# NeurAI-Lab/biHomE

Hardware: AMD Instinct MI355X
Metric: training image-pairs/s (128x128 patch, bs=64 per GPU, full step: fwd+bwd+Adam) (higher is better)
Workload: dtype f32

## Files before the change

### bihome_amd/csrc/conv3x3.hip

```cpp
#include "common.h"
#include "conv3x3_args.h"
#include <type_traits>

#ifndef C3_X3_PIPE
#define C3_X3_PIPE 0
#endif

#ifndef C3_BN32_WAVES
#define C3_BN32_WAVES 2
#endif

#ifdef BH_TUNING
__device__ unsigned long long g_c3_ts[8 * 16384];
#define C3_STAMP(tile, k) do { if (a.dbg_ts && threadIdx.x == 0 && (tile) < 16384) { g_c3_ts[(tile) * 8 + (k)] = wall_clock64();          \
        if ((k) == 1 || (k) == 2) g_c3_ts[(tile) * 8 + 4 + (k)] = __builtin_readcyclecounter(); } } while (0)
#else
#define C3_STAMP(tile, k) do { } while (0)
#endif

constexpr int C3_HALO_BYTES = 8 * 200 * 16;
constexpr int C3_B_BYTES = 8192;
constexpr int C3_LDS_BYTES = 2 * C3_HALO_BYTES + 2 * C3_B_BYTES;

template <int BN, int SUBT, int TM, bool MAP4 = false>
// ... 635 lines not shown
            for (int r = 0; r < 16; ++r) acc[i][r] = __builtin_ldexpf(acc[i][r], f16_kout);
    }
    double s1, s2;
    int img, g;
    c3_epilogue<BN, SUBT, TM, MAP4>(a, acc, bx, n0, wm, wn, wh, l31, kh2, s1, s2, img, g, AMX);
    if (a.bn_sums) {
        if (a.stat_acc) { S1 += s1; S2 += s2; Sbx = bx; if (g < Sg) { Sg = g; Simg = img; } }
        else c3_stats_merge<BN, 0>(a, smem, s1, s2, img, g, bx, n0, wave, lane, tid);
    }
#ifdef BH_TUNING
    if (a.dbg_ts) asm volatile("s_waitcnt vmcnt(0)" ::: "memory");
#endif
    __syncthreads();
    C3_STAMP(bx * gridDim.y + blockIdx.y, 3);
    }
    if (a.bn_sums && a.stat_acc) c3_stats_merge<BN, 0>(a, smem, S1, S2, Simg, Sg, Sbx, n0, wave, lane, tid);
    if (a.amax_out) {
        const float m = wave_max(AMX);
        if (lane == 0) atomicMax(a.amax_out + ((blockIdx.x * 4 + wave) % BH_AMAX_SLOTS) * BH_AMAX_STRIDE, __builtin_bit_cast(unsigned, m));
    }
}

constexpr int C3_MIN_BLOCKS = 256;
BH_KNOB(g_c3_noload, 0); BH_KNOB(g_c3_dbg_nch, -1); BH_KNOB(g_c3_subt, 2); BH_KNOB(g_c3_tpb, 2); BH_KNOB(g_c3_stamp, 0); BH_KNOB(g_c3_desync, 0); BH_KNOB(g_c3_walk32, 1); BH_KNOB(g_c3_pc, 1); BH_KNOB(g_c3_wt64, 512); BH_KNOB(g_c3_wt32, 512);
#ifdef BH_TUNING
extern "C" int bh_debug_read_c3_stamps(unsigned long long* out, int n) {
    if (n > 16384) n = 16384;
    return (int)hipMemcpyFromSymbol(out, HIP_SYMBOL(g_c3_ts), (size_t)n * 8 * sizeof(unsigned long long), 0, hipMemcpyDeviceToHost);
}
void bh_conv3x3_tune(int disable, int min_blocks) {
    (void)min_blocks;
    if (disable >= 500 && disable < 1000) { g_c3_stamp = disable - 500; return; }
    if (disable >= 200 && disable < 264) { g_c3_desync = disable - 200; return; }
    if (disable == 300 || disable == 301) { g_c3_walk32 = disable - 300; return; }
    if (disable >= 2000 && disable < 6000) { g_c3_wt64 = disable - 2000; return; }
    if (disable >= 6000 && disable < 10000) { g_c3_wt32 = disable - 6000; return; }
    if (disable == 310 || disable == 311) { g_c3_pc = disable - 310; return; }
    if (disable <= -100) { g_c3_dbg_nch = -100 - disable - 1; return; }
    if (disable >= 400 && disable < 464) { g_c3_noload = disable - 400; return; }
    if (disable >= 20 && disable < 24) { g_c3_tpb = disable - 20; return; }
    if (disable >= 11 && disable <= 13) { g_c3_subt = disable - 10; return; }
}
#endif

int bh_conv3x3_try(const float* src, const float* w, const float* bias, float* out, const bh_conv_desc* d, int dgrad,
                   int accumulate, hipStream_t stream, int* taken, double* bn_sums, int groups, const float* res, int relu,
                   const bh_bn_reduce* bnr, const bh_bn_in* bni) {
    *taken = 0;
    if ((d->route & BH_ROUTE_GENERIC_CONV) || d->transposed || d->kh != 3 || d->kw != 3 || d->stride != 1 || d->pad != 1 || d->in_nchw ||
        d->out_nchw || d->precision < 0 || d->precision > 4)
        return d->w_layout ? BH_E_UNSUPPORTED : 0;
    if (d->w_layout != 0 && ((d->w_layout == 2) != (d->precision == 2) || (d->w_layout == 3) != (d->precision == 3) ||
                             (d->w_layout == 4) != (d->precision == 4))) return BH_E_BADARG;
    if (d->w_layout == 4 && !d->a_bound) return BH_E_BADARG;
    const bool map4 = d->Hi == 4 && d->Wi == 4 && d->Ho == 4 && d->Wo == 4 && d->N % 4 == 0 && (d->w_layout >= 2 && d->w_layout <= 4) &&
                      d->Co % 64 == 0 && d->Ci % 64 == 0 && !bni && (!bn_sums || (groups >= 1 && d->N % groups == 0 && (d->N / groups) % 4 == 0));
    if (!map4 && (d->Hi % 8 || d->Wi % 8 || d->Ho != d->Hi || d->Wo != d->Wi)) return d->w_layout ? BH_E_UNSUPPORTED : 0;
    const int Kc = dgrad ? d->Co : d->Ci, Nn = dgrad ? d->Ci : d->Co;
    if (Kc % 32 || Nn % 32) return d->w_layout ? BH_E_UNSUPPORTED : 0;
    const int bn_tile = (Nn % 64) ? 32 : 64;
// ... 40 lines not shown
    if (bn_sums && !map4 && !(d->route & BH_ROUTE_C3_ONE_POSITION) && groups >= 1 && a.subtiles % (subt * groups) == 0) {
        const int ppg = a.subtiles / (subt * groups);
        int t = a.tpb;
        const long long wtarget = (x3 && bn_tile == 64) ? g_c3_wt64 : (x3 ? g_c3_wt32 : 2048);
        while (ppg % (t * 2) == 0 && (ppg / t > 1024 || (long long)(ppg / t) * groups * grid.y > wtarget) && t < 64) t *= 2;
        if (ppg % t == 0 && (t > 1 || a.tpb == 1)) {
            if (t != a.tpb) { a.tpb = t; grid.x = (a.gx_total + t - 1) / t; }
            a.stat_acc = 1;
        }
    }
    if (x3 && !map4 && a.tpb == 1 && !bn_sums && g_c3_walk32 && !(d->route & BH_ROUTE_C3_ONE_POSITION)) {
        const long long target = bn_tile == 32 ? 1024 : 512;
        int t = 1;
        while (a.gx_total % (t * 2) == 0 && (long long)(a.gx_total / (t * 2)) * grid.y >= target && t < 64) t *= 2;
        if (t > 1) { a.tpb = t; grid.x = a.gx_total / t; }
    }
    if (!(d->route & BH_ROUTE_HALO_SMALL) && (int)((map4 ? a.subtiles : (a.subtiles + 1) / 2) * grid.y) < (map4 ? C3_MIN_BLOCKS / 2 : C3_MIN_BLOCKS))
        return d->w_layout ? BH_E_UNSUPPORTED : 0;
    a.NW = Nn / 32;
    if (bni) {
        if (!x3 || dgrad || !bni->table || bni->groups < 1 || d->N % bni->groups || (long long)bni->groups * Kc * 8 > 4096) return BH_E_UNSUPPORTED;
        a.bni = bni->table; a.bni_relu = bni->relu; a.bni_groups = bni->groups; a.bni_ipg = d->N / bni->groups;
    }
    if (f16 && !map4 && bn_tile == 64 && !(d->route & (BH_ROUTE_C3_TILE_WG | BH_ROUTE_C3_ONE_SUBTILE | BH_ROUTE_C3_ONE_POSITION)) && g_c3_pc) {
        C3Args b = a;
        b.det = (d->route & BH_ROUTE_DETERMINISTIC) ? 1 : 0; b.dbg_noload = g_c3_noload; b.dbg_ts = g_c3_stamp;
        const int st = bh_conv3x3_pc_launch(b, dgrad, bni ? bni->table : nullptr, bni ? bni->groups : 0, bni ? bni->relu : 0, (d->route & BH_ROUTE_C3_PC) != 0, stream);
        if (st != BH_E_UNSUPPORTED) { if (st == BH_OK) *taken = 1; return st; }
    }
    if (bh_query("conv3x3_halo_kernel<%s,%d,%s,%d,%s,%s,%s,%d,%s,%s>", dgrad ? "true" : "false", bn_tile, bf16 ? "true" : "false", subt,
                 packed ? "true" : "false", x3 ? "true" : "false", bni ? "true" : "false", np, map4 ? "true" : "false", f16 ? "true" : "false")) {
        *taken = 1;
        return BH_OK;
    }
    static unsigned long long attr_devs = 0;
    typedef void (*kern_t)(C3Args);
#define C3_ROW(P) conv3x3_halo_kernel<false, 64, false, 2, P>, conv3x3_halo_kernel<true, 64, false, 2, P>,   \
                  conv3x3_halo_kernel<false, 32, false, 2, P>, conv3x3_halo_kernel<true, 32, false, 2, P>,   \
                  conv3x3_halo_kernel<false, 64, true, 2, P>,  conv3x3_halo_kernel<true, 64, true, 2, P>,    \
                  conv3x3_halo_kernel<false, 32, true, 2, P>,  conv3x3_halo_kernel<true, 32, true, 2, P>,    \
                  conv3x3_halo_kernel<false, 64, false, 1, P>, conv3x3_halo_kernel<true, 64, false, 1, P>,   \
                  conv3x3_halo_kernel<false, 64, true, 1, P>,  conv3x3_halo_kernel<true, 64, true, 1, P>
#define C3_XROW(NP_, F_) conv3x3_halo_kernel<false, 64, false, 2, true, true, false, NP_, false, F_>, conv3x3_halo_kernel<true, 64, false, 2, true, true, false, NP_, false, F_>,  \
                     conv3x3_halo_kernel<false, 32, false, 2, true, true, false, NP_, false, F_>, conv3x3_halo_kernel<true, 32, false, 2, true, true, false, NP_, false, F_>,  \
                     conv3x3_halo_kernel<false, 64, false, 1, true, true, false, NP_, false, F_>, conv3x3_halo_kernel<true, 64, false, 1, true, true, false, NP_, false, F_>,  \
                     conv3x3_halo_kernel<false, 64, false, 2, true, true, true, NP_, false, F_>, conv3x3_halo_kernel<false, 32, false, 2, true, true, true, NP_, false, F_>,   \
                     conv3x3_halo_kernel<false, 64, false, 1, true, true, true, NP_, false, F_>
// ... 148 lines not shown
```

### bihome_amd/csrc/conv3x3_pc.hip

```cpp
#include "conv3x3_args.h"
#include <type_traits>

namespace {
constexpr int PC_HPL = 200;
constexpr int PC_PS = PC_HPL * 16 + 32;
constexpr int PC_PIECE = 4 * PC_PS;
constexpr int PC_STAGE = 2 * PC_PIECE;
constexpr int PC_BTAP = 8192;
constexpr int PC_BROW = 3 * PC_BTAP;
constexpr int PC_OFF_B = 2 * PC_STAGE;
constexpr int PC_OFF_EPI = PC_OFF_B + 3 * PC_BROW;
constexpr int PC_EPI_BYTES = 128 * 64 * 4;
constexpr int PC_OFF_RED = PC_OFF_EPI + PC_EPI_BYTES;
constexpr int PC_RED_BYTES = 4 * 128 * 8;
constexpr int PC_LDS = PC_OFF_RED + PC_RED_BYTES;
constexpr unsigned PC_XOOB = 0x80000000u;

#ifdef BH_TUNING
__device__ unsigned long long g_pc_ts[12 * 160 * 2];
#define PC_BARRIER()                                                                                                    \
    do {                                                                                                                \
        const bool st_ = a.dbg_ts && blockIdx.x == (unsigned)(a.dbg_ts - 1) && (tid & 63) == 0;                        \
        if (st_ && pc_nb < 160) g_pc_ts[(wave * 160 + pc_nb) * 2] = __builtin_readcyclecounter();                       \
        asm volatile("s_waitcnt lgkmcnt(0)\n\ts_barrier" ::: "memory");                                                \
        if (st_ && pc_nb < 160) g_pc_ts[(wave * 160 + pc_nb) * 2 + 1] = __builtin_readcyclecounter();                   \
        ++pc_nb;                                                                                                        \
    } while (0)
#else
#define PC_BARRIER() asm volatile("s_waitcnt lgkmcnt(0)\n\ts_barrier" ::: "memory")
#endif
#ifndef PC_EMU
#define PC_EMU 0
#endif
#define PC_H_ASM 0
#define PC_BARRIER_VM() asm volatile("s_waitcnt vmcnt(0)\n\ts_waitcnt lgkmcnt(0)\n\ts_barrier" ::: "memory")

__device__ __forceinline__ unsigned pc_amax_reduce(unsigned v) {
#pragma unroll
    for (int off = 8; off > 0; off >>= 1) { const unsigned o = (unsigned)__shfl_xor((int)v, off, 64); v = o > v ? o : v; }
    return (unsigned)__builtin_amdgcn_readfirstlane((int)v);
}

__device__ __forceinline__ void pc_decode(const C3Args& a, int g, int& img, int& ty, int& tx) {
    if (a.tpi_shift >= 0) { img = g >> a.tpi_shift; const int t = g & (a.tiles_per_img - 1); ty = t >> a.tx_shift; tx = t & (a.tiles_x - 1); }
    else { img = g / a.tiles_per_img; const int t = g - img * a.tiles_per_img; ty = t / a.tiles_x; tx = t - ty * a.tiles_x; }
}

template <bool DGRAD, bool BNI, int EM>
__global__ void __launch_bounds__(768) conv3x3_pc_kernel(C3Args a) {
    extern __shared__ __attribute__((aligned(16))) char smem[];
    const int tid = threadIdx.x, lane = tid & 63;
    const int wave = __builtin_amdgcn_readfirstlane(tid >> 6);
    const int NY = a.Nn >> 6;
    const int total = a.gx_total * NY;
    const int wt0 = blockIdx.x * a.tpb;
    const int Tw = min(a.tpb, total - wt0);
    const int nch = a.Kc >> 5;
    const int K = Tw * nch;
    const int R = K * 3;
#ifdef BH_TUNING
    int pc_nb = 0;
#endif

    auto wait_vm = [&](int n) {
#define PC_W(k) case k: asm volatile("s_waitcnt vmcnt(" #k ")" ::: "memory"); break;
        switch (n < 0 ? 0 : (n > 48 ? 48 : n)) {
            PC_W(0) PC_W(1) PC_W(2) PC_W(3) PC_W(4) PC_W(5) PC_W(6) PC_W(7) PC_W(8) PC_W(9) PC_W(10) PC_W(11) PC_W(12) PC_W(13) PC_W(14) PC_W(15)
            PC_W(16) PC_W(17) PC_W(18) PC_W(19) PC_W(20) PC_W(21) PC_W(22) PC_W(23) PC_W(24) PC_W(25) PC_W(26) PC_W(27) PC_W(28) PC_W(29) PC_W(30)
            PC_W(31) PC_W(32) PC_W(33) PC_W(34) PC_W(35) PC_W(36) PC_W(37) PC_W(38) PC_W(39) PC_W(40) PC_W(41) PC_W(42) PC_W(43) PC_W(44) PC_W(45)
            PC_W(46) PC_W(47) PC_W(48)
        }
#undef PC_W
    };

    if (wave < 4) {
        const int l31 = lane & 31, kh2 = lane >> 5;
        const int wm = wave & 1, wn = wave >> 1;
        const int sr_ = c3_strip_row(l31 >> 2);
        const char* const aL = smem + kh2 * PC_PS + (wm * 100 + sr_ * 10 + (l31 & 3)) * 16;
        const char* const bL = smem + PC_OFF_B + wn * 4096 + lane * 16;
        int eoff[4];
#pragma unroll
        for (int rq = 0; rq < 4; ++rq) eoff[rq] = PC_OFF_EPI + ((wm * 64 + c3_strip_row(2 * rq + kh2) * 8) * 64 + wn * 32 + l31) * 4;
        uint4 FA0[2][2], FB0[2], FA1[2][2], FB1[2];
        f32x16 acc[2];
#ifdef BH_TUNING
        const int dbg = a.dbg_noload;
#else
        constexpr int dbg = 0;
#endif
#define PC_LD_A(A_, ap, s2, i_, pc_) A_[i_][pc_] = *reinterpret_cast<const uint4*>((ap) + (pc_) * PC_PIECE + 2 * (s2) * PC_PS + (i_) * 64)
#define PC_LD_B(B_, bp, s2, pc_) B_[pc_] = *reinterpret_cast<const uint4*>((bp) + ((pc_) * 2 + (s2)) * 1024)
#define PC_LOADH(A_, B_, ap, bp, s2)                                                                                    \
    do {                                                                                                                \
        PC_LD_A(A_, ap, s2, 0, 1); PC_LD_B(B_, bp, s2, 0); PC_LD_A(A_, ap, s2, 1, 1);                                   \
        PC_LD_A(A_, ap, s2, 0, 0); PC_LD_B(B_, bp, s2, 1); PC_LD_A(A_, ap, s2, 1, 0);                                   \
    } while (0)
#define PC_STEP(ACC, AV, BV, LD)                                                                                        \
    do {                                                                                                                \
        ACC = c3_mfma16<true>(AV, BV, ACC);                                                                             \
        LD;                                                                                                             \
        __builtin_amdgcn_sched_barrier(0);                                                                              \
    } while (0)
#define PC_HALF(UA, UB, LA, LB, ap, bp, s2)                                                                             \
    do {                                                                                                                \
        PC_STEP(acc[0], UA[0][1], UB[0], PC_LD_A(LA, ap, s2, 0, 1));                                                    \
        PC_STEP(acc[1], UA[1][1], UB[0], PC_LD_B(LB, bp, s2, 0));                                                       \
        PC_STEP(acc[0], UA[0][0], UB[1], PC_LD_A(LA, ap, s2, 1, 1));                                                    \
        PC_STEP(acc[1], UA[1][0], UB[1], PC_LD_A(LA, ap, s2, 0, 0));                                                    \
        PC_STEP(acc[0], UA[0][0], UB[0], PC_LD_B(LB, bp, s2, 1));                                                       \
        PC_STEP(acc[1], UA[1][0], UB[0], PC_LD_A(LA, ap, s2, 1, 0));                                                    \
    } while (0)
#define PC_HALF_PRE(UA, UB, LA, LB, ap, bp, s2)                                                                         \
    do {                                                                                                                \
        PC_LOADH(LA, LB, ap, bp, s2);                                                                                   \
        __builtin_amdgcn_sched_barrier(0);                                                                              \
        PC_STEP(acc[0], UA[0][1], UB[0], (void)0);                                                                      \
        PC_STEP(acc[1], UA[1][1], UB[0], (void)0);                                                                      \
        PC_STEP(acc[0], UA[0][0], UB[1], (void)0);                                                                      \
        PC_STEP(acc[1], UA[1][0], UB[1], (void)0);                                                                      \
        PC_STEP(acc[0], UA[0][0], UB[0], (void)0);                                                                      \
        PC_STEP(acc[1], UA[1][0], UB[0], (void)0);                                                                      \
    } while (0)
        PC_BARRIER();
        PC_LOADH(FA0, FB0, aL, bL, 0);
#if PC_EMU
        PC_LOADH(FA1, FB1, aL, bL, 1);
#undef PC_LD_B
#define PC_LD_B(B_, bp, s2, pc_) (void)0
#if PC_EMU >= 2
#undef PC_LD_A
#if PC_EMU == 2
#define PC_LD_A(A_, ap, s2, i_, pc_) (void)0
#else
#define PC_LD_A(A_, ap, s2, i_, pc_) do { if ((i_) == 0) A_[i_][pc_] = *reinterpret_cast<const uint4*>((ap) + (pc_) * PC_PIECE + 2 * (s2) * PC_PS + (i_) * 64); } while (0)
#endif
#endif
#endif
        int kap = 0;
        for (int ti = 0; ti < Tw; ++ti) {
#pragma unroll
            for (int i = 0; i < 2; ++i)
#pragma unroll
                for (int r = 0; r < 16; ++r) acc[i][r] = 0.0f;
            for (int c = 0; c < nch; ++c, ++kap) {
                const int par = kap & 1;
                const bool more = kap + 1 < K;
#pragma unroll
                for (int row = 0; row < 3; ++row) {
                    const char* const rp = aL + par * PC_STAGE + row * 160;
                    const char* const sp = bL + row * PC_BROW;
                    const char* const nrp = row < 2 ? rp + 160 : (more ? aL + (par ^ 1) * PC_STAGE : rp);
                    const char* const nsp = row < 2 ? sp + PC_BROW : bL;
                    if (dbg & 1) { PC_BARRIER(); continue; }
#pragma unroll
                    for (int t = 0; t < 3; ++t) {
                        if (t < 2) PC_HALF(FA0, FB0, FA1, FB1, rp + t * 16, sp + t * PC_BTAP, 1);
                        else {
                            PC_HALF_PRE(FA0, FB0, FA1, FB1, rp + t * 16, sp + t * PC_BTAP, 1);
                            PC_BARRIER();
                        }
                        if (t < 2) PC_HALF(FA1, FB1, FA0, FB0, rp + (t + 1) * 16, sp + (t + 1) * PC_BTAP, 0);
                        else PC_HALF(FA1, FB1, FA0, FB0, nrp, nsp, 0);
                    }
                }
            }
            asm volatile("s_nop 15\n\ts_nop 15" : "+v"(acc[0]), "+v"(acc[1]));
#pragma unroll
            for (int i = 0; i < 2; ++i)
#pragma unroll
                for (int r = 0; r < 16; ++r)
                    *reinterpret_cast<float*>(smem + eoff[r >> 2] + (4 * i + (r & 3)) * 256) = acc[i][r];
        }
        PC_BARRIER();
        PC_BARRIER();
        PC_BARRIER();
        PC_BARRIER();
#undef PC_HALF_PRE
#undef PC_HALF
#undef PC_STEP
#undef PC_LOADH
#undef PC_LD_A
#undef PC_LD_B
        return;
    }

    if (wave < 7) {
        __builtin_amdgcn_s_setprio(2);
        const int ht = tid - 256;
        const int plane = ht & 3;
        const __amdgpu_buffer_rsrc_t rsA = __builtin_amdgcn_make_buffer_rsrc(const_cast<float*>(a.Src), 0, a.src_bytes, 0x00020000);
        const __amdgpu_buffer_rsrc_t rsT = __builtin_amdgcn_make_buffer_rsrc(const_cast<float*>(BNI ? a.bni : a.Src), 0,
                                                                              BNI ? (unsigned)(a.bni_groups * a.Kc * 8) : 0u, 0x00020000);
        constexpr int NR = 5;
        const int lo0 = plane * PC_PS + (ht >> 2) * 16;
// ... 136 lines not shown
        PC_BARRIER();
        PC_BARRIER();
        PC_BARRIER();
#undef PC_H_ISSUE_ALL
#undef PC_H_CHUNK
        return;
    }

    if (wave < 8) {
        const __amdgpu_buffer_rsrc_t rsB = __builtin_amdgcn_make_buffer_rsrc(const_cast<float*>(a.Wt), 0, a.w_bytes, 0x00020000);
#ifdef BH_TUNING
        const bool doff = a.dbg_noload & 8;
#else
        constexpr bool doff = false;
#endif
        auto dma_num = [&](int r) {
            const int kp = r / 3, row = r - kp * 3, ti_ = kp / nch, c_ = kp - ti_ * nch;
            const int ny = (wt0 + ti_) / a.gx_total;
#pragma unroll
            for (int t = 0; t < 3; ++t)
#pragma unroll
                for (int piece = 0; piece < 8; ++piece) {
                    const unsigned so = (unsigned)(((c_ * 9 + row * 3 + t) * a.NW + ny * 2) * 4096 + piece * 1024);
                    __builtin_amdgcn_raw_ptr_buffer_load_lds(rsB, (lds_void_ptr)(smem + PC_OFF_B + row * PC_BROW + t * PC_BTAP + piece * 1024), 16,
                                                             (unsigned)lane * 16u, so, 0, 0);
                }
        };
        int pro = 0;
        if (!doff) { dma_num(0); if (R > 1) { dma_num(1); ++pro; } if (R > 2) { dma_num(2); ++pro; } }
        wait_vm(24 * pro);
        PC_BARRIER();
        for (int rho = 0; rho < R; ++rho) {
            int nd = 0;
            if (rho >= 1 && rho + 2 < R && !doff) { dma_num(rho + 2); nd = 24; }
            wait_vm(rho == 0 ? ((R > 2 && !doff) ? 24 : 0) : nd);
            PC_BARRIER();
        }
        PC_BARRIER();
        PC_BARRIER();
        PC_BARRIER();
        PC_BARRIER();
        return;
    }

    {
        __builtin_amdgcn_s_setprio(1);
        const int ew = wave - 8;
        const int cq = lane & 15, pl = lane >> 4;
        const __amdgpu_buffer_rsrc_t rsO = __builtin_amdgcn_make_buffer_rsrc(a.Out, 0, a.out_bytes, 0x00020000);
        const __amdgpu_buffer_rsrc_t rsR = __builtin_amdgcn_make_buffer_rsrc(const_cast<float*>(a.res ? a.res : a.Out), 0, a.out_bytes, 0x00020000);
        const __amdgpu_buffer_rsrc_t rsZ = __builtin_amdgcn_make_buffer_rsrc(const_cast<float*>(a.bnr_z ? a.bnr_z : a.Out), 0, a.out_bytes, 0x00020000);
        const __amdgpu_buffer_rsrc_t rsY = __builtin_amdgcn_make_buffer_rsrc(const_cast<float*>(a.bnr_y ? a.bnr_y : a.Out), 0, a.out_bytes, 0x00020000);
        constexpr bool stats = EM & 1, use_ext = EM & 2, rd_z = EM & 4, rd_y = EM & 8;
        const bool rd_res = a.res != nullptr;
        const unsigned nn4 = (unsigned)a.Nn * 4u;
#ifdef BH_TUNING
        const bool eoff_ = a.dbg_noload & 16;
#else
        constexpr bool eoff_ = false;
#endif

        unsigned tbase[2] = {0u, 0u}, fbase[2] = {0u, 0u};
        bool tvalid[2] = {false, false}, fvalid[2] = {false, false};
        float4 bv = make_float4(0.f, 0.f, 0.f, 0.f);
        float4 r_invstd = bv, r_cx0 = bv, r_sc = bv, r_sh = bv;
        int cur_grp = -1, cur_n0 = 0;
        double S1[4] = {0.0, 0.0, 0.0, 0.0}, S2[4] = {0.0, 0.0, 0.0, 0.0};
        float amx = 0.0f;
        bool have = false;
        int pend_grp = 0, pend_n0 = 0;
        bool pending = false;
        auto stash = [&]() {
            double* const red = reinterpret_cast<double*>(smem + PC_OFF_RED);
#pragma unroll
            for (int e = 0; e < 4; ++e) {
                double s1 = S1[e], s2 = S2[e];
                s1 += __shfl_xor(s1, 16, 64); s1 += __shfl_xor(s1, 32, 64);
                s2 += __shfl_xor(s2, 16, 64); s2 += __shfl_xor(s2, 32, 64);
                if (pl == 0) { red[(ew * 64 + cq * 4 + e) * 2] = s1; red[(ew * 64 + cq * 4 + e) * 2 + 1] = s2; }
                S1[e] = 0.0; S2[e] = 0.0;
            }
            pend_grp = cur_grp; pend_n0 = cur_n0; pending = true; have = false;
        };
        auto commit = [&]() {
            if (!pending) return;
            if (ew == 0) {
                const double* const red = reinterpret_cast<const double*>(smem + PC_OFF_RED);
#pragma unroll
                for (int q = 0; q < 2; ++q) {
                    const int idx = q * 64 + lane;
                    const double tot = ((red[idx] + red[128 + idx]) + red[256 + idx]) + red[384 + idx];
                    bh_acc_add(&a.bn_sums[bn_sum_index(0, a.groups, pend_grp, a.Nn, pend_n0 + (idx >> 1), idx & 1)], tot, a.det);
                }
            }
            pending = false;
        };
        auto tile_geom = [&](int wt, unsigned (&base)[2], bool (&valid)[2], int& grp, int& n0) {
            const int ny_ = wt / a.gx_total, bx = wt - ny_ * a.gx_total;
            n0 = ny_ * 64; grp = 0;
#pragma unroll
            for (int s_ = 0; s_ < 2; ++s_) {
                const int g = bx * 2 + s_;
                int img, ty, tx;
                pc_decode(a, g < a.subtiles ? g : 0, img, ty, tx);
                valid[s_] = g < a.subtiles;
                base[s_] = ((unsigned)((img * a.H + ty * 8) * a.W + tx * 8) * (unsigned)a.Nn + (unsigned)n0) * 4u;
                if (s_ == 0) grp = img / a.imgs_per_group;
            }
        };
        auto f_tile = [&](int wt) { int g_, n_; tile_geom(wt, fbase, fvalid, g_, n_); };
        auto e_tile = [&](int wt) {
            int grp, n0;
            tile_geom(wt, tbase, tvalid, grp, n0);
            if (stats && have && (grp != cur_grp || n0 != cur_n0)) stash();
            if (grp != cur_grp || n0 != cur_n0) {
                cur_grp = grp; cur_n0 = n0;
                const int n = n0 + cq * 4;
                bv = a.bias ? *reinterpret_cast<const float4*>(a.bias + n) : make_float4(0.f, 0.f, 0.f, 0.f);
                if (rd_z) {
                    float isd[4], cx[4], sc[4], sh[4];
                    const double rows = (double)a.bnr_rows;
#pragma unroll
                    for (int e = 0; e < 4; ++e) {
                        const double mu = bn_sum_total(a.bnr_stats, a.groups, grp, a.Nn, n + e, 0, a.det) / rows;
                        double var = bn_sum_total(a.bnr_stats, a.groups, grp, a.Nn, n + e, 1, a.det) / rows - mu * mu;
                        if (var < 0) var = 0;
                        const float mean = (float)mu;
                        isd[e] = 1.0f / sqrtf((float)var + a.bnr_eps);
                        sc[e] = (a.bnr_gamma ? a.bnr_gamma[n + e] : 1.f) * isd[e];
                        sh[e] = (a.bnr_beta ? a.bnr_beta[n + e] : 0.f) - mean * sc[e];
                        cx[e] = -mean * isd[e];
                    }
                    r_invstd = make_float4(isd[0], isd[1], isd[2], isd[3]); r_cx0 = make_float4(cx[0], cx[1], cx[2], cx[3]);
                    r_sc = make_float4(sc[0], sc[1], sc[2], sc[3]); r_sh = make_float4(sh[0], sh[1], sh[2], sh[3]);
                }
            }
        };
        float4 pf_a[4], pf_z[4], pf_y[4];
        constexpr int nld = (use_ext ? 1 : 0) + (rd_z ? 1 : 0) + (rd_y ? 1 : 0);
        const unsigned voff = (unsigned)((ew >> 1) * a.W + ((ew & 1) << 2) + pl) * nn4 + (unsigned)cq * 16u;
        const unsigned rowstep2 = 2u * (unsigned)a.W * nn4;
        const char* const epi_l = smem + PC_OFF_EPI + ew * 1024 + lane * 16;
        const __amdgpu_buffer_rsrc_t rsA_ = rd_res ? rsR : rsO;
        auto epi_fetch = [&](auto Q, int idx) {
            constexpr int q = decltype(Q)::value;
            if (nld == 0 || !((idx >> 2) ? fvalid[1] : fvalid[0])) return;
            const unsigned so = ((idx >> 2) ? fbase[1] : fbase[0]) + (unsigned)(idx & 3) * rowstep2;
            if constexpr (use_ext) pf_a[q] = __builtin_bit_cast(float4, __builtin_amdgcn_raw_buffer_load_b128(rsA_, voff, so, 0));
            if constexpr (rd_z) pf_z[q] = __builtin_bit_cast(float4, __builtin_amdgcn_raw_buffer_load_b128(rsZ, voff, so, 0));
            if constexpr (rd_y) pf_y[q] = __builtin_bit_cast(float4, __builtin_amdgcn_raw_buffer_load_b128(rsY, voff, so, 0));
        };
        int kout = 0;
        auto epi_run = [&](auto Q, int idx) {
            constexpr int q = decltype(Q)::value;
            if (!((idx >> 2) ? tvalid[1] : tvalid[0])) return;
            const unsigned so = ((idx >> 2) ? tbase[1] : tbase[0]) + (unsigned)(idx & 3) * rowstep2;
            const float4 av = *reinterpret_cast<const float4*>(epi_l + idx * 4096);
            const float4 z0 = make_float4(0.f, 0.f, 0.f, 0.f);
            const float4 o = use_ext ? pf_a[q] : z0, zz = rd_z ? pf_z[q] : z0, yy = rd_y ? pf_y[q] : z0;
            const float accv[4] = {av.x, av.y, av.z, av.w}, bb[4] = {bv.x, bv.y, bv.z, bv.w};
            const float oo[4] = {o.x, o.y, o.z, o.w};
            const float z4[4] = {zz.x, zz.y, zz.z, zz.w}, y4[4] = {yy.x, yy.y, yy.z, yy.w};
            const float isd[4] = {r_invstd.x, r_invstd.y, r_invstd.z, r_invstd.w}, cx[4] = {r_cx0.x, r_cx0.y, r_cx0.z, r_cx0.w};
            const float sc[4] = {r_sc.x, r_sc.y, r_sc.z, r_sc.w}, sh[4] = {r_sh.x, r_sh.y, r_sh.z, r_sh.w};
            float out[4];
            const bool do_relu = a.relu != 0, mask_on = rd_z && a.bnr_relu;
#pragma unroll
            for (int e = 0; e < 4; ++e) {
                float v = __builtin_ldexpf(accv[e], kout) + bb[e];
                if constexpr (use_ext) v += oo[e];
                v = do_relu ? fmaxf(v, 0.0f) : v;
                out[e] = v;
                if constexpr (stats) {
                    float vm = v, t = v;
                    if constexpr (rd_z) {
                        const float yv = rd_y ? y4[e] : __builtin_fmaf(z4[e], sc[e], sh[e]);
                        vm = (mask_on && !(yv > 0.f)) ? 0.f : v;
                        t = __builtin_fmaf(z4[e], isd[e], cx[e]);
                        amx = fmaxf(amx, fabsf(vm));
                    }
                    S1[e] += (double)vm;
                    S2[e] = __builtin_fma((double)vm, (double)t, S2[e]);
                }
            }
            const __attribute__((ext_vector_type(4))) unsigned ov =
                __builtin_bit_cast(__attribute__((ext_vector_type(4))) unsigned, make_float4(out[0], out[1], out[2], out[3]));
            __builtin_amdgcn_raw_buffer_store_b128(ov, rsO, voff, so, 0);
            asm volatile("s_nop 3" :: "v"(ov));
            have = true;
        };
        using Q0 = std::integral_constant<int, 0>; using Q1 = std::integral_constant<int, 1>; using Q2 = std::integral_constant<int, 2>;
        using Q3 = std::integral_constant<int, 3>;
        const int nph = 3 * nch;
        const int grp = ew >> 1;
        const int nA = grp ? (nph - 1) / 2 : nph / 2;
        constexpr int UB = 4, NB = 2;
        const int BPP = (NB + nA - 1) / nA;
        auto run_batch = [&](int b) {
            const int i0 = b * UB;
            epi_run(Q0{}, i0 + 0); epi_run(Q1{}, i0 + 1); epi_run(Q2{}, i0 + 2); epi_run(Q3{}, i0 + 3);
        };
        auto fetch_batch = [&](int b) {
            const int i0 = b * UB;
            epi_fetch(Q0{}, i0 + 0); epi_fetch(Q1{}, i0 + 1); epi_fetch(Q2{}, i0 + 2); epi_fetch(Q3{}, i0 + 3);
        };
        auto step_batch = [&](int b, int nxt) {
            run_batch(b);
            if (nld == 0) return;
            if (b + 1 < NB) fetch_batch(b + 1);
            else if (nxt >= 0) { f_tile(nxt); fetch_batch(0); }
        };

        if (!eoff_) {
            const unsigned* const wrec = reinterpret_cast<const unsigned*>(a.Wt) + (a.w_bytes >> 2);
            const unsigned wv = lane < 16 ? wrec[lane] : 0u;
            const unsigned rec_ = lane < BH_AMAX_SLOTS ? a.amax_src[lane * BH_AMAX_STRIDE] : 0u;
            kout = -(bh_f16_scale_exp(pc_amax_reduce(wv)) + bh_f16_scale_exp(pc_amax_reduce(rec_)));
            asm volatile("" :: "s"(kout) : "memory");
            f_tile(wt0);
// ... 21 lines not shown
        commit();
        PC_BARRIER();
        if (!eoff_) {
            for (int b = 0; b < NB; ++b) step_batch(b, -1);
            if (stats) stash();
        }
        PC_BARRIER();
        commit();
        if (rd_z && a.amax_out) {
            const float m = wave_max(amx);
            if (lane == 0) atomicMax(a.amax_out + ((blockIdx.x * 4 + ew) % BH_AMAX_SLOTS) * BH_AMAX_STRIDE, __builtin_bit_cast(unsigned, m));
        }
    }
}
}

#ifdef BH_TUNING
extern "C" int bh_debug_read_pc_stamps(unsigned long long* out) {
    return (int)hipMemcpyFromSymbol(out, HIP_SYMBOL(g_pc_ts), sizeof(unsigned long long) * 12 * 160 * 2, 0, hipMemcpyDeviceToHost);
}
#endif

int bh_conv3x3_pc_launch(C3Args& a, int dgrad, const float* bni_table, int bni_groups, int bni_relu, bool force, hipStream_t stream) {
    if (a.Kc % 32 || a.Nn % 64 || a.subtiles < 1) return BH_E_UNSUPPORTED;
    const long long sub_per_group = (long long)a.imgs_per_group * a.tiles_per_img;
    if ((a.bn_sums || a.bnr_z) && (sub_per_group % 2)) return BH_E_UNSUPPORTED;
    if (a.accumulate && a.res) return BH_E_UNSUPPORTED;
    if (a.bnr_z && !a.bn_sums) return BH_E_UNSUPPORTED;
    if (bni_table) {
        if (dgrad || bni_groups < 1 || a.N % bni_groups || ((long long)(a.N / bni_groups) * a.tiles_per_img) % 2) return BH_E_UNSUPPORTED;
        a.bni = bni_table; a.bni_groups = bni_groups; a.bni_relu = bni_relu; a.bni_ipg = a.N / bni_groups;
    }
    const int em = (a.bn_sums ? 1 : 0) | ((a.accumulate || a.res) ? 2 : 0) | (a.bnr_z ? 4 : 0) | ((a.bnr_z && a.bnr_relu && a.bnr_y) ? 8 : 0);
    typedef void (*kern_t)(C3Args);
    struct Row { int dgrad, bni, em; kern_t fn; };
#define PC_ROW(D, B, E) {D, B, E, conv3x3_pc_kernel<(D) != 0, (B) != 0, E>}
    static const Row rows[] = {PC_ROW(0, 0, 0), PC_ROW(0, 0, 1), PC_ROW(0, 0, 2), PC_ROW(0, 1, 0), PC_ROW(0, 1, 1),
                               PC_ROW(1, 0, 0), PC_ROW(1, 0, 1), PC_ROW(1, 0, 2), PC_ROW(1, 0, 5), PC_ROW(1, 0, 7), PC_ROW(1, 0, 13), PC_ROW(1, 0, 15)};
#undef PC_ROW
    constexpr int NROWS = sizeof(rows) / sizeof(rows[0]);
    kern_t fn = nullptr;
    for (int i = 0; i < NROWS; ++i)
        if (rows[i].dgrad == (dgrad ? 1 : 0) && rows[i].bni == (bni_table ? 1 : 0) && rows[i].em == em) fn = rows[i].fn;
    if (!fn) return BH_E_UNSUPPORTED;
    a.gx_total = (a.subtiles + 1) / 2;
    const long long total = (long long)a.gx_total * (a.Nn / 64);
    const int cus = 256;
    const int T = (int)((total + cus - 1) / cus);
    if (!force && (em & 14) && dgrad && T > 1) return BH_E_UNSUPPORTED;
    const int grid = (int)((total + T - 1) / T);
    a.tpb = T;
    a.NW = a.Nn / 32;
    if (bh_query("conv3x3_pc_kernel<%s,%s,%d>", dgrad ? "true" : "false", bni_table ? "true" : "false", em)) return BH_OK;
    static unsigned long long attr_devs = 0;
    if (bh_device_once(attr_devs)) {
        for (int i = 0; i < NROWS; ++i) {
            hipError_t e = hipFuncSetAttribute(reinterpret_cast<const void*>(rows[i].fn), hipFuncAttributeMaxDynamicSharedMemorySize, PC_LDS);
            if (e != hipSuccess) return (int)e;
        }
    }
    hipLaunchKernelGGL(fn, dim3(grid), dim3(768), PC_LDS, stream, a);
    BH_LAUNCH_CHECK();
    return BH_OK;
}
```

Baseline: 5326.

## Add 32-channel tile variant of producer-consumer conv3x3 kernel

Templates the producer-consumer conv3x3 kernel on output-channel tile width (64 or 32) and routes f16 3x3 convs with 32 in/out channels (forward only, no BN sums) to it instead of the older halo kernel. The 32-wide variant loads all weights once into LDS, uses one MFMA accumulator per wave with the waves split spatially, and adjusts the epilogue mapping and reductions. It is enabled by default through a new knob. It adds more kernel instantiations and a separate LDS layout, and it may run with lower MFMA density per wave.

```diff
diff --git a/bihome_amd/csrc/conv3x3.hip b/bihome_amd/csrc/conv3x3.hip
--- a/bihome_amd/csrc/conv3x3.hip
+++ b/bihome_amd/csrc/conv3x3.hip
@@ -681,7 +681,10 @@
 }
 
 constexpr int C3_MIN_BLOCKS = 256;
-BH_KNOB(g_c3_noload, 0); BH_KNOB(g_c3_dbg_nch, -1); BH_KNOB(g_c3_subt, 2); BH_KNOB(g_c3_tpb, 2); BH_KNOB(g_c3_stamp, 0); BH_KNOB(g_c3_desync, 0); BH_KNOB(g_c3_walk32, 1); BH_KNOB(g_c3_pc, 1); BH_KNOB(g_c3_wt64, 512); BH_KNOB(g_c3_wt32, 512);
+#ifndef C3_PC32
+#define C3_PC32 1
+#endif
+BH_KNOB(g_c3_noload, 0); BH_KNOB(g_c3_dbg_nch, -1); BH_KNOB(g_c3_subt, 2); BH_KNOB(g_c3_tpb, 2); BH_KNOB(g_c3_stamp, 0); BH_KNOB(g_c3_desync, 0); BH_KNOB(g_c3_walk32, 1); BH_KNOB(g_c3_pc, 1); BH_KNOB(g_c3_pc32, C3_PC32); BH_KNOB(g_c3_wt64, 512); BH_KNOB(g_c3_wt32, 512);
 #ifdef BH_TUNING
 extern "C" int bh_debug_read_c3_stamps(unsigned long long* out, int n) {
     if (n > 16384) n = 16384;
@@ -695,6 +698,7 @@
     if (disable >= 2000 && disable < 6000) { g_c3_wt64 = disable - 2000; return; }
     if (disable >= 6000 && disable < 10000) { g_c3_wt32 = disable - 6000; return; }
     if (disable == 310 || disable == 311) { g_c3_pc = disable - 310; return; }
+    if (disable == 312 || disable == 313) { g_c3_pc32 = disable - 312; return; }
     if (disable <= -100) { g_c3_dbg_nch = -100 - disable - 1; return; }
     if (disable >= 400 && disable < 464) { g_c3_noload = disable - 400; return; }
     if (disable >= 20 && disable < 24) { g_c3_tpb = disable - 20; return; }
@@ -781,7 +785,8 @@
         if (!x3 || dgrad || !bni->table || bni->groups < 1 || d->N % bni->groups || (long long)bni->groups * Kc * 8 > 4096) return BH_E_UNSUPPORTED;
         a.bni = bni->table; a.bni_relu = bni->relu; a.bni_groups = bni->groups; a.bni_ipg = d->N / bni->groups;
     }
-    if (f16 && !map4 && bn_tile == 64 && !(d->route & (BH_ROUTE_C3_TILE_WG | BH_ROUTE_C3_ONE_SUBTILE | BH_ROUTE_C3_ONE_POSITION)) && g_c3_pc) {
+    if (f16 && !map4 && (bn_tile == 64 || g_c3_pc32) && !(d->route & (BH_ROUTE_C3_TILE_WG | BH_ROUTE_C3_ONE_SUBTILE | BH_ROUTE_C3_ONE_POSITION)) &&
+        g_c3_pc) {
         C3Args b = a;
         b.det = (d->route & BH_ROUTE_DETERMINISTIC) ? 1 : 0; b.dbg_noload = g_c3_noload; b.dbg_ts = g_c3_stamp;
         const int st = bh_conv3x3_pc_launch(b, dgrad, bni ? bni->table : nullptr, bni ? bni->groups : 0, bni ? bni->relu : 0, (d->route & BH_ROUTE_C3_PC) != 0, stream);
diff --git a/bihome_amd/csrc/conv3x3_pc.hip b/bihome_amd/csrc/conv3x3_pc.hip
--- a/bihome_amd/csrc/conv3x3_pc.hip
+++ b/bihome_amd/csrc/conv3x3_pc.hip
@@ -6,14 +6,16 @@
 constexpr int PC_PS = PC_HPL * 16 + 32;
 constexpr int PC_PIECE = 4 * PC_PS;
 constexpr int PC_STAGE = 2 * PC_PIECE;
-constexpr int PC_BTAP = 8192;
-constexpr int PC_BROW = 3 * PC_BTAP;
-constexpr int PC_OFF_B = 2 * PC_STAGE;
-constexpr int PC_OFF_EPI = PC_OFF_B + 3 * PC_BROW;
-constexpr int PC_EPI_BYTES = 128 * 64 * 4;
-constexpr int PC_OFF_RED = PC_OFF_EPI + PC_EPI_BYTES;
-constexpr int PC_RED_BYTES = 4 * 128 * 8;
-constexpr int PC_LDS = PC_OFF_RED + PC_RED_BYTES;
+template <int NT> struct PcL {
+    static constexpr int BTAP = NT * 128;
+    static constexpr int BROW = 3 * BTAP;
+    static constexpr int OFF_B = 2 * PC_STAGE;
+    static constexpr int OFF_EPI = OFF_B + 3 * BROW;
+    static constexpr int EPI_BYTES = 128 * NT * 4;
+    static constexpr int OFF_RED = OFF_EPI + EPI_BYTES;
+    static constexpr int RED_BYTES = 4 * NT * 2 * 8;
+    static constexpr int LDS = OFF_RED + RED_BYTES;
+};
 constexpr unsigned PC_XOOB = 0x80000000u;
 
 #ifdef BH_TUNING
@@ -46,12 +48,15 @@
     else { img = g / a.tiles_per_img; const int t = g - img * a.tiles_per_img; ty = t / a.tiles_x; tx = t - ty * a.tiles_x; }
 }
 
-template <bool DGRAD, bool BNI, int EM>
+template <bool DGRAD, bool BNI, int EM, int NT>
 __global__ void __launch_bounds__(768) conv3x3_pc_kernel(C3Args a) {
+    static_assert(NT == 64 || NT == 32, "64- or 32-channel tile");
+    constexpr bool C32 = NT == 32;
+    using L = PcL<NT>;
     extern __shared__ __attribute__((aligned(16))) char smem[];
     const int tid = threadIdx.x, lane = tid & 63;
     const int wave = __builtin_amdgcn_readfirstlane(tid >> 6);
-    const int NY = a.Nn >> 6;
+    const int NY = a.Nn / NT;
     const int total = a.gx_total * NY;
     const int wt0 = blockIdx.x * a.tpb;
     const int Tw = min(a.tpb, total - wt0);
@@ -75,15 +80,16 @@
 
     if (wave < 4) {
         const int l31 = lane & 31, kh2 = lane >> 5;
-        const int wm = wave & 1, wn = wave >> 1;
+        const int wm = C32 ? wave >> 1 : wave & 1, wn = C32 ? 0 : wave >> 1, wh = C32 ? wave & 1 : 0;
         const int sr_ = c3_strip_row(l31 >> 2);
-        const char* const aL = smem + kh2 * PC_PS + (wm * 100 + sr_ * 10 + (l31 & 3)) * 16;
-        const char* const bL = smem + PC_OFF_B + wn * 4096 + lane * 16;
+        const char* const aL = smem + kh2 * PC_PS + (wm * 100 + sr_ * 10 + wh * 4 + (l31 & 3)) * 16;
+        const char* const bL = smem + L::OFF_B + wn * 4096 + lane * 16;
         int eoff[4];
 #pragma unroll
-        for (int rq = 0; rq < 4; ++rq) eoff[rq] = PC_OFF_EPI + ((wm * 64 + c3_strip_row(2 * rq + kh2) * 8) * 64 + wn * 32 + l31) * 4;
-        uint4 FA0[2][2], FB0[2], FA1[2][2], FB1[2];
-        f32x16 acc[2];
+        for (int rq = 0; rq < 4; ++rq) eoff[rq] = L::OFF_EPI + ((wm * 64 + c3_strip_row(2 * rq + kh2) * 8 + wh * 4) * NT + wn * 32 + l31) * 4;
+        constexpr int NF = C32 ? 1 : 2;
+        uint4 FA0[NF][2], FB0[2], FA1[NF][2], FB1[2];
+        f32x16 acc[NF];
 #ifdef BH_TUNING
         const int dbg = a.dbg_noload;
 #else
@@ -104,26 +110,41 @@
     } while (0)
 #define PC_HALF(UA, UB, LA, LB, ap, bp, s2)                                                                             \
     do {                                                                                                                \
-        PC_STEP(acc[0], UA[0][1], UB[0], PC_LD_A(LA, ap, s2, 0, 1));                                                    \
-        PC_STEP(acc[1], UA[1][1], UB[0], PC_LD_B(LB, bp, s2, 0));                                                       \
-        PC_STEP(acc[0], UA[0][0], UB[1], PC_LD_A(LA, ap, s2, 1, 1));                                                    \
-        PC_STEP(acc[1], UA[1][0], UB[1], PC_LD_A(LA, ap, s2, 0, 0));                                                    \
-        PC_STEP(acc[0], UA[0][0], UB[0], PC_LD_B(LB, bp, s2, 1));                                                       \
-        PC_STEP(acc[1], UA[1][0], UB[0], PC_LD_A(LA, ap, s2, 1, 0));                                                    \
+        if constexpr (C32) {                                     \
+            PC_STEP(acc[0], UA[0][1], UB[0], (PC_LD_A(LA, ap, s2, 0, 1), PC_LD_B(LB, bp, s2, 0)));                      \
+            PC_STEP(acc[0], UA[0][0], UB[1], PC_LD_A(LA, ap, s2, 0, 0));                                                \
+            PC_STEP(acc[0], UA[0][0], UB[0], PC_LD_B(LB, bp, s2, 1));                                                   \
+        } else {                                                                                                        \
+            PC_STEP(acc[0], UA[0][1], UB[0], PC_LD_A(LA, ap, s2, 0, 1));                                                \
+            PC_STEP(acc[1], UA[1][1], UB[0], PC_LD_B(LB, bp, s2, 0));                                                   \
+            PC_STEP(acc[0], UA[0][0], UB[1], PC_LD_A(LA, ap, s2, 1, 1));                                                \
+            PC_STEP(acc[1], UA[1][0], UB[1], PC_LD_A(LA, ap, s2, 0, 0));                                                \
+            PC_STEP(acc[0], UA[0][0], UB[0], PC_LD_B(LB, bp, s2, 1));                                                   \
+            PC_STEP(acc[1], UA[1][0], UB[0], PC_LD_A(LA, ap, s2, 1, 0));                                                \
+        }                                                                                                               \
     } while (0)
 #define PC_HALF_PRE(UA, UB, LA, LB, ap, bp, s2)                                                                         \
     do {                                                                                                                \
-        PC_LOADH(LA, LB, ap, bp, s2);                                                                                   \
-        __builtin_amdgcn_sched_barrier(0);                                                                              \
-        PC_STEP(acc[0], UA[0][1], UB[0], (void)0);                                                                      \
-        PC_STEP(acc[1], UA[1][1], UB[0], (void)0);                                                                      \
-        PC_STEP(acc[0], UA[0][0], UB[1], (void)0);                                                                      \
-        PC_STEP(acc[1], UA[1][0], UB[1], (void)0);                                                                      \
-        PC_STEP(acc[0], UA[0][0], UB[0], (void)0);                                                                      \
-        PC_STEP(acc[1], UA[1][0], UB[0], (void)0);                                                                      \
+        if constexpr (C32) {                                                                                            \
+            PC_LD_A(LA, ap, s2, 0, 1); PC_LD_B(LB, bp, s2, 0); PC_LD_A(LA, ap, s2, 0, 0); PC_LD_B(LB, bp, s2, 1);       \
+            __builtin_amdgcn_sched_barrier(0);                                                                          \
+            PC_STEP(acc[0], UA[0][1], UB[0], (void)0);                                                                  \
+            PC_STEP(acc[0], UA[0][0], UB[1], (void)0);                                                                  \
+            PC_STEP(acc[0], UA[0][0], UB[0], (void)0);                                                                  \
+        } else {                                                                                                        \
+            PC_LOADH(LA, LB, ap, bp, s2);                                                                               \
+            __builtin_amdgcn_sched_barrier(0);                                                                          \
+            PC_STEP(acc[0], UA[0][1], UB[0], (void)0);                                                                  \
+            PC_STEP(acc[1], UA[1][1], UB[0], (void)0);                                                                  \
+            PC_STEP(acc[0], UA[0][0], UB[1], (void)0);                                                                  \
+            PC_STEP(acc[1], UA[1][0], UB[1], (void)0);                                                                  \
+            PC_STEP(acc[0], UA[0][0], UB[0], (void)0);                                                                  \
+            PC_STEP(acc[1], UA[1][0], UB[0], (void)0);                                                                  \
+        }                                                                                                               \
     } while (0)
         PC_BARRIER();
-        PC_LOADH(FA0, FB0, aL, bL, 0);
+        if constexpr (C32) { PC_LD_A(FA0, aL, 0, 0, 1); PC_LD_B(FB0, bL, 0, 0); PC_LD_A(FA0, aL, 0, 0, 0); PC_LD_B(FB0, bL, 0, 1); }
+        else PC_LOADH(FA0, FB0, aL, bL, 0);
 #if PC_EMU
         PC_LOADH(FA1, FB1, aL, bL, 1);
 #undef PC_LD_B
@@ -140,7 +161,7 @@
         int kap = 0;
         for (int ti = 0; ti < Tw; ++ti) {
 #pragma unroll
-            for (int i = 0; i < 2; ++i)
+            for (int i = 0; i < NF; ++i)
 #pragma unroll
                 for (int r = 0; r < 16; ++r) acc[i][r] = 0.0f;
             for (int c = 0; c < nch; ++c, ++kap) {
@@ -149,28 +170,29 @@
 #pragma unroll
                 for (int row = 0; row < 3; ++row) {
                     const char* const rp = aL + par * PC_STAGE + row * 160;
-                    const char* const sp = bL + row * PC_BROW;
+                    const char* const sp = bL + row * L::BROW;
                     const char* const nrp = row < 2 ? rp + 160 : (more ? aL + (par ^ 1) * PC_STAGE : rp);
-                    const char* const nsp = row < 2 ? sp + PC_BROW : bL;
+                    const char* const nsp = row < 2 ? sp + L::BROW : bL;
                     if (dbg & 1) { PC_BARRIER(); continue; }
 #pragma unroll
                     for (int t = 0; t < 3; ++t) {
-                        if (t < 2) PC_HALF(FA0, FB0, FA1, FB1, rp + t * 16, sp + t * PC_BTAP, 1);
+                        if (t < 2) PC_HALF(FA0, FB0, FA1, FB1, rp + t * 16, sp + t * L::BTAP, 1);
                         else {
-                            PC_HALF_PRE(FA0, FB0, FA1, FB1, rp + t * 16, sp + t * PC_BTAP, 1);
+                            PC_HALF_PRE(FA0, FB0, FA1, FB1, rp + t * 16, sp + t * L::BTAP, 1);
                             PC_BARRIER();
                         }
-                        if (t < 2) PC_HALF(FA1, FB1, FA0, FB0, rp + (t + 1) * 16, sp + (t + 1) * PC_BTAP, 0);
+                        if (t < 2) PC_HALF(FA1, FB1, FA0, FB0, rp + (t + 1) * 16, sp + (t + 1) * L::BTAP, 0);
                         else PC_HALF(FA1, FB1, FA0, FB0, nrp, nsp, 0);
                     }
                 }
             }
-            asm volatile("s_nop 15\n\ts_nop 15" : "+v"(acc[0]), "+v"(acc[1]));
-#pragma unroll
-            for (int i = 0; i < 2; ++i)
+            if constexpr (C32) asm volatile("s_nop 15\n\ts_nop 15" : "+v"(acc[0]));
+            else asm volatile("s_nop 15\n\ts_nop 15" : "+v"(acc[0]), "+v"(acc[NF - 1]));
+#pragma unroll
+            for (int i = 0; i < NF; ++i)
 #pragma unroll
                 for (int r = 0; r < 16; ++r)
-                    *reinterpret_cast<float*>(smem + eoff[r >> 2] + (4 * i + (r & 3)) * 256) = acc[i][r];
+                    *reinterpret_cast<float*>(smem + eoff[r >> 2] + (4 * i + (r & 3)) * (NT * 4)) = acc[i][r];
         }
         PC_BARRIER();
         PC_BARRIER();
@@ -353,10 +375,26 @@
 #pragma unroll
                 for (int piece = 0; piece < 8; ++piece) {
                     const unsigned so = (unsigned)(((c_ * 9 + row * 3 + t) * a.NW + ny * 2) * 4096 + piece * 1024);
-                    __builtin_amdgcn_raw_ptr_buffer_load_lds(rsB, (lds_void_ptr)(smem + PC_OFF_B + row * PC_BROW + t * PC_BTAP + piece * 1024), 16,
+                    __builtin_amdgcn_raw_ptr_buffer_load_lds(rsB, (lds_void_ptr)(smem + L::OFF_B + row * L::BROW + t * L::BTAP + piece * 1024), 16,
                                                              (unsigned)lane * 16u, so, 0, 0);
                 }
         };
+        if constexpr (C32) {
+            if (!doff) {
+#pragma unroll
+                for (int q = 0; q < 36; ++q)
+                    __builtin_amdgcn_raw_ptr_buffer_load_lds(rsB, (lds_void_ptr)(smem + L::OFF_B + q * 1024), 16, (unsigned)lane * 16u,
+                                                             (unsigned)q * 1024u, 0, 0);
+            }
+            wait_vm(0);
+            PC_BARRIER();
+            for (int rho = 0; rho < R; ++rho) PC_BARRIER();
+            PC_BARRIER();
+            PC_BARRIER();
+            PC_BARRIER();
+            PC_BARRIER();
+            return;
+        }
         int pro = 0;
         if (!doff) { dma_num(0); if (R > 1) { dma_num(1); ++pro; } if (R > 2) { dma_num(2); ++pro; } }
         wait_vm(24 * pro);
@@ -377,7 +415,8 @@
     {
         __builtin_amdgcn_s_setprio(1);
         const int ew = wave - 8;
-        const int cq = lane & 15, pl = lane >> 4;
+        constexpr int NQ = NT / 4;
+        const int cq = lane % NQ, pl = lane / NQ;
         const __amdgpu_buffer_rsrc_t rsO = __builtin_amdgcn_make_buffer_rsrc(a.Out, 0, a.out_bytes, 0x00020000);
         const __amdgpu_buffer_rsrc_t rsR = __builtin_amdgcn_make_buffer_rsrc(const_cast<float*>(a.res ? a.res : a.Out), 0, a.out_bytes, 0x00020000);
         const __amdgpu_buffer_rsrc_t rsZ = __builtin_amdgcn_make_buffer_rsrc(const_cast<float*>(a.bnr_z ? a.bnr_z : a.Out), 0, a.out_bytes, 0x00020000);
@@ -402,13 +441,13 @@
         int pend_grp = 0, pend_n0 = 0;
         bool pending = false;
         auto stash = [&]() {
-            double* const red = reinterpret_cast<double*>(smem + PC_OFF_RED);
+            double* const red = reinterpret_cast<double*>(smem + L::OFF_RED);
 #pragma unroll
             for (int e = 0; e < 4; ++e) {
                 double s1 = S1[e], s2 = S2[e];
-                s1 += __shfl_xor(s1, 16, 64); s1 += __shfl_xor(s1, 32, 64);
-                s2 += __shfl_xor(s2, 16, 64); s2 += __shfl_xor(s2, 32, 64);
-                if (pl == 0) { red[(ew * 64 + cq * 4 + e) * 2] = s1; red[(ew * 64 + cq * 4 + e) * 2 + 1] = s2; }
+#pragma unroll
+                for (int off = NQ; off < 64; off <<= 1) { s1 += __shfl_xor(s1, off, 64); s2 += __shfl_xor(s2, off, 64); }
+                if (pl == 0) { red[(ew * NT + cq * 4 + e) * 2] = s1; red[(ew * NT + cq * 4 + e) * 2 + 1] = s2; }
                 S1[e] = 0.0; S2[e] = 0.0;
             }
             pend_grp = cur_grp; pend_n0 = cur_n0; pending = true; have = false;
@@ -416,11 +455,11 @@
         auto commit = [&]() {
             if (!pending) return;
             if (ew == 0) {
-                const double* const red = reinterpret_cast<const double*>(smem + PC_OFF_RED);
-#pragma unroll
-                for (int q = 0; q < 2; ++q) {
+                const double* const red = reinterpret_cast<const double*>(smem + L::OFF_RED);
+#pragma unroll
+                for (int q = 0; q < NT / 32; ++q) {
                     const int idx = q * 64 + lane;
-                    const double tot = ((red[idx] + red[128 + idx]) + red[256 + idx]) + red[384 + idx];
+                    const double tot = ((red[idx] + red[2 * NT + idx]) + red[4 * NT + idx]) + red[6 * NT + idx];
                     bh_acc_add(&a.bn_sums[bn_sum_index(0, a.groups, pend_grp, a.Nn, pend_n0 + (idx >> 1), idx & 1)], tot, a.det);
                 }
             }
@@ -428,7 +467,7 @@
         };
         auto tile_geom = [&](int wt, unsigned (&base)[2], bool (&valid)[2], int& grp, int& n0) {
             const int ny_ = wt / a.gx_total, bx = wt - ny_ * a.gx_total;
-            n0 = ny_ * 64; grp = 0;
+            n0 = ny_ * NT; grp = 0;
 #pragma unroll
             for (int s_ = 0; s_ < 2; ++s_) {
                 const int g = bx * 2 + s_;
@@ -469,14 +508,16 @@
         };
         float4 pf_a[4], pf_z[4], pf_y[4];
         constexpr int nld = (use_ext ? 1 : 0) + (rd_z ? 1 : 0) + (rd_y ? 1 : 0);
-        const unsigned voff = (unsigned)((ew >> 1) * a.W + ((ew & 1) << 2) + pl) * nn4 + (unsigned)cq * 16u;
-        const unsigned rowstep2 = 2u * (unsigned)a.W * nn4;
-        const char* const epi_l = smem + PC_OFF_EPI + ew * 1024 + lane * 16;
+        constexpr int UPS = C32 ? 2 : 4;
+        const unsigned voff = C32 ? (unsigned)(ew * a.W + pl) * nn4 + (unsigned)cq * 16u
+                                  : (unsigned)((ew >> 1) * a.W + ((ew & 1) << 2) + pl) * nn4 + (unsigned)cq * 16u;
+        const unsigned rowstep2 = (C32 ? 4u : 2u) * (unsigned)a.W * nn4;
+        const char* const epi_l = smem + L::OFF_EPI + ew * 1024 + lane * 16;
         const __amdgpu_buffer_rsrc_t rsA_ = rd_res ? rsR : rsO;
         auto epi_fetch = [&](auto Q, int idx) {
             constexpr int q = decltype(Q)::value;
-            if (nld == 0 || !((idx >> 2) ? fvalid[1] : fvalid[0])) return;
-            const unsigned so = ((idx >> 2) ? fbase[1] : fbase[0]) + (unsigned)(idx & 3) * rowstep2;
+            if (nld == 0 || !((idx / UPS) ? fvalid[1] : fvalid[0])) return;
+            const unsigned so = ((idx / UPS) ? fbase[1] : fbase[0]) + (unsigned)(idx % UPS) * rowstep2;
             if constexpr (use_ext) pf_a[q] = __builtin_bit_cast(float4, __builtin_amdgcn_raw_buffer_load_b128(rsA_, voff, so, 0));
             if constexpr (rd_z) pf_z[q] = __builtin_bit_cast(float4, __builtin_amdgcn_raw_buffer_load_b128(rsZ, voff, so, 0));
             if constexpr (rd_y) pf_y[q] = __builtin_bit_cast(float4, __builtin_amdgcn_raw_buffer_load_b128(rsY, voff, so, 0));
@@ -484,8 +525,8 @@
         int kout = 0;
         auto epi_run = [&](auto Q, int idx) {
             constexpr int q = decltype(Q)::value;
-            if (!((idx >> 2) ? tvalid[1] : tvalid[0])) return;
-            const unsigned so = ((idx >> 2) ? tbase[1] : tbase[0]) + (unsigned)(idx & 3) * rowstep2;
+            if (!((idx / UPS) ? tvalid[1] : tvalid[0])) return;
+            const unsigned so = ((idx / UPS) ? tbase[1] : tbase[0]) + (unsigned)(idx % UPS) * rowstep2;
             const float4 av = *reinterpret_cast<const float4*>(epi_l + idx * 4096);
             const float4 z0 = make_float4(0.f, 0.f, 0.f, 0.f);
             const float4 o = use_ext ? pf_a[q] : z0, zz = rd_z ? pf_z[q] : z0, yy = rd_y ? pf_y[q] : z0;
@@ -525,7 +566,7 @@
         const int nph = 3 * nch;
         const int grp = ew >> 1;
         const int nA = grp ? (nph - 1) / 2 : nph / 2;
-        constexpr int UB = 4, NB = 2;
+        constexpr int UB = 4, NB = C32 ? 1 : 2;
         const int BPP = (NB + nA - 1) / nA;
         auto run_batch = [&](int b) {
             const int i0 = b * UB;
@@ -593,7 +634,8 @@
 #endif
 
 int bh_conv3x3_pc_launch(C3Args& a, int dgrad, const float* bni_table, int bni_groups, int bni_relu, bool force, hipStream_t stream) {
-    if (a.Kc % 32 || a.Nn % 64 || a.subtiles < 1) return BH_E_UNSUPPORTED;
+    const bool c32 = a.Nn % 64 != 0;
+    if (a.subtiles < 1 || (c32 ? (a.Kc != 32 || a.Nn != 32 || dgrad || a.bn_sums) : a.Kc % 32 != 0)) return BH_E_UNSUPPORTED;
     const long long sub_per_group = (long long)a.imgs_per_group * a.tiles_per_img;
     if ((a.bn_sums || a.bnr_z) && (sub_per_group % 2)) return BH_E_UNSUPPORTED;
     if (a.accumulate && a.res) return BH_E_UNSUPPORTED;
@@ -604,18 +646,21 @@
     }
     const int em = (a.bn_sums ? 1 : 0) | ((a.accumulate || a.res) ? 2 : 0) | (a.bnr_z ? 4 : 0) | ((a.bnr_z && a.bnr_relu && a.bnr_y) ? 8 : 0);
     typedef void (*kern_t)(C3Args);
-    struct Row { int dgrad, bni, em; kern_t fn; };
-#define PC_ROW(D, B, E) {D, B, E, conv3x3_pc_kernel<(D) != 0, (B) != 0, E>}
-    static const Row rows[] = {PC_ROW(0, 0, 0), PC_ROW(0, 0, 1), PC_ROW(0, 0, 2), PC_ROW(0, 1, 0), PC_ROW(0, 1, 1),
-                               PC_ROW(1, 0, 0), PC_ROW(1, 0, 1), PC_ROW(1, 0, 2), PC_ROW(1, 0, 5), PC_ROW(1, 0, 7), PC_ROW(1, 0, 13), PC_ROW(1, 0, 15)};
+    struct Row { int nt, dgrad, bni, em; kern_t fn; };
+#define PC_ROW(T, D, B, E) {T, D, B, E, conv3x3_pc_kernel<(D) != 0, (B) != 0, E, T>}
+    static const Row rows[] = {PC_ROW(64, 0, 0, 0), PC_ROW(64, 0, 0, 1), PC_ROW(64, 0, 0, 2), PC_ROW(64, 0, 1, 0), PC_ROW(64, 0, 1, 1),
+                               PC_ROW(64, 1, 0, 0), PC_ROW(64, 1, 0, 1), PC_ROW(64, 1, 0, 2), PC_ROW(64, 1, 0, 5), PC_ROW(64, 1, 0, 7),
+                               PC_ROW(64, 1, 0, 13), PC_ROW(64, 1, 0, 15),
+                               PC_ROW(32, 0, 0, 0), PC_ROW(32, 0, 0, 2), PC_ROW(32, 0, 1, 0)};
 #undef PC_ROW
     constexpr int NROWS = sizeof(rows) / sizeof(rows[0]);
+    const int nt = c32 ? 32 : 64;
     kern_t fn = nullptr;
     for (int i = 0; i < NROWS; ++i)
-        if (rows[i].dgrad == (dgrad ? 1 : 0) && rows[i].bni == (bni_table ? 1 : 0) && rows[i].em == em) fn = rows[i].fn;
+        if (rows[i].nt == nt && rows[i].dgrad == (dgrad ? 1 : 0) && rows[i].bni == (bni_table ? 1 : 0) && rows[i].em == em) fn = rows[i].fn;
     if (!fn) return BH_E_UNSUPPORTED;
     a.gx_total = (a.subtiles + 1) / 2;
-    const long long total = (long long)a.gx_total * (a.Nn / 64);
+    const long long total = (long long)a.gx_total * (a.Nn / nt);
     const int cus = 256;
     const int T = (int)((total + cus - 1) / cus);
     if (!force && (em & 14) && dgrad && T > 1) return BH_E_UNSUPPORTED;
@@ -626,11 +671,12 @@
     static unsigned long long attr_devs = 0;
     if (bh_device_once(attr_devs)) {
         for (int i = 0; i < NROWS; ++i) {
-            hipError_t e = hipFuncSetAttribute(reinterpret_cast<const void*>(rows[i].fn), hipFuncAttributeMaxDynamicSharedMemorySize, PC_LDS);
+            hipError_t e = hipFuncSetAttribute(reinterpret_cast<const void*>(rows[i].fn), hipFuncAttributeMaxDynamicSharedMemorySize,
+                                               rows[i].nt == 32 ? PcL<32>::LDS : PcL<64>::LDS);
             if (e != hipSuccess) return (int)e;
         }
     }
-    hipLaunchKernelGGL(fn, dim3(grid), dim3(768), PC_LDS, stream, a);
+    hipLaunchKernelGGL(fn, dim3(grid), dim3(768), c32 ? PcL<32>::LDS : PcL<64>::LDS, stream, a);
     BH_LAUNCH_CHECK();
     return BH_OK;
 }
```

Result: slower. 5245, median of 2 (-1.5%).
